# xshazwar/noize-job

Hardware: AMD Instinct MI355X
Metric: Mcells/s 4096^2 simplex13oct->Gauss5x17->FlowMap->Erosion; %HBM roofline @1/8GPU (higher is better)
Workload: dtype f32

## Files before the change

noize_job_amd/csrc/nz_filter.hip:

```cpp
#include <cstdlib>

#include "nz_internal.hpp"

namespace {

constexpr int CT = 256;
constexpr int TW = 128;
__host__ __device__ constexpr int conv_hx(int H) { return (H + 3) & ~3; }
constexpr int TH = 64;

__device__ __forceinline__ int clampi(int v, int lo, int hi) { return v < lo ? lo : (v > hi ? hi : v); }

__device__ __forceinline__ int xcd_tile_index() {
    int bid = blockIdx.x;
    int nb = gridDim.x, q = nb >> 3, r = nb & 7;
    int x = bid & 7, k = bid >> 3;
    return x * q + (x < r ? x : r) + k;
}

__device__ __forceinline__ void tile_origin(const nz_geom &g, int OW, int OH, int &ox0, int &oz0) {
    int tiles_x = (g.cols + OW - 1) / OW;
    int bid = xcd_tile_index();
    int by = bid / tiles_x;
    int bx = bid - by * tiles_x;
    ox0 = bx * OW;
    oz0 = g.or0 + by * OH;
}

constexpr int RB = 8;

__device__ __forceinline__ float dpp_prev(float v) {
    return __builtin_bit_cast(float, __builtin_amdgcn_mov_dpp(__builtin_bit_cast(int, v), 0x138, 0xf, 0xf, true));
}
__device__ __forceinline__ float dpp_next(float v) {
    return __builtin_bit_cast(float, __builtin_amdgcn_mov_dpp(__builtin_bit_cast(int, v), 0x130, 0xf, 0xf, true));
}

#ifdef NZ_CONV_PROBE
__device__ unsigned long long *nz_probe_buf = nullptr;
#define NZ_PB_PARAM , unsigned long long *nz_pb
#define NZ_PB_ARG , nz_pb
#define NZ_PB_INIT unsigned long long *nz_pb = threadIdx.x == 0 ? nz_probe_buf : nullptr
#define NZ_PROBE(slot, val)                                              \
    do {                                                                 \
        if (nz_pb) nz_pb[(size_t)blockIdx.x * 24 + (slot)] = (val);      \
    } while (0)
#define NZ_PROBE_T(slot) NZ_PROBE(slot, __builtin_amdgcn_s_memrealtime())
#else
#define NZ_PB_PARAM
#define NZ_PB_ARG
#define NZ_PB_INIT
#define NZ_PROBE(slot, val)
#define NZ_PROBE_T(slot)
#endif

constexpr int conv_waves(int ks, int nt, int rbt) { return rbt < RB ? 4 : ks == 5 ? 6 : (nt >= 512 || ks >= 7) ? 4 : 6; }
constexpr int conv_nbuf(int o) { return o >= 2 ? 1 : 2; }

typedef unsigned nz_v4u __attribute__((ext_vector_type(4)));
constexpr int NZ_AUX_SC1 = 16;
__device__ __forceinline__ float4 load16_sc1(const float *base, size_t float_off) {
    __amdgpu_buffer_rsrc_t r = __builtin_amdgcn_make_buffer_rsrc(const_cast<float *>(base), 0, -1, 0x00020000);
    nz_v4u t = __builtin_amdgcn_raw_buffer_load_b128(r, (int)(float_off * 4), 0, NZ_AUX_SC1);
    return make_float4(__uint_as_float(t.x), __uint_as_float(t.y), __uint_as_float(t.z), __uint_as_float(t.w));
}
__device__ __forceinline__ void store16_sc1(float *base, size_t float_off, float4 v) {
    __amdgpu_buffer_rsrc_t r = __builtin_amdgcn_make_buffer_rsrc(base, 0, -1, 0x00020000);
    nz_v4u t = {__float_as_uint(v.x), __float_as_uint(v.y), __float_as_uint(v.z), __float_as_uint(v.w)};
    __builtin_amdgcn_raw_buffer_store_b128(t, r, (int)(float_off * 4), 0, NZ_AUX_SC1);
}
__device__ __forceinline__ float load4_sc1(const float *base, size_t float_off) {
    __amdgpu_buffer_rsrc_t r = __builtin_amdgcn_make_buffer_rsrc(const_cast<float *>(base), 0, -1, 0x00020000);
    return __uint_as_float(__builtin_amdgcn_raw_buffer_load_b32(r, (int)(float_off * 4), 0, NZ_AUX_SC1));
}
__device__ __forceinline__ void store4_sc1(float *base, size_t float_off, float v) {
    __amdgpu_buffer_rsrc_t r = __builtin_amdgcn_make_buffer_rsrc(base, 0, -1, 0x00020000);
    __builtin_amdgcn_raw_buffer_store_b32(__float_as_uint(v), r, (int)(float_off * 4), 0, NZ_AUX_SC1);
}

template <bool FAST>
__device__ __forceinline__ float tap_acc(float total, float v, float k) {
    return FAST ? __builtin_fmaf(v, k, total) : total + v * k;
}
template <bool FAST, bool SEED>
__device__ __forceinline__ float tap_first(float v, float k) {
    return FAST ? __builtin_fmaf(v, k, 0.0f) : SEED ? 0.0f + v * k : v * k;
}

template <int KS, bool UNIT, int NT, bool SC1, bool FAST, int RBT>
__device__ __forceinline__ void conv_tile(const float *__restrict__ src, float *__restrict__ dst, const nz_geom &g,
                                          const nz_kernel_taps &taps, int T, int aligned, int ox0, int oz0,
                                          float4 *s_edge_raw NZ_PB_PARAM) {
    constexpr int O = (KS - 1) / 2;
    constexpr int WN = 4 + 2 * O;
    constexpr int ZN = RBT + 2 * O;
    constexpr int TH = NT / 32 * RBT;
    static_assert(O <= RBT, "a block's window reaches into the neighbouring blocks only");
    constexpr int NBUF = conv_nbuf(O);
    float4 (*s_edge)[TH / RBT][2][O][TW / 4] = reinterpret_cast<float4 (*)[TH / RBT][2][O][TW / 4]>(s_edge_raw);

    const int tid = threadIdx.x, cg = tid & 31, rb = tid >> 5;
    const int H = T * O, HX = conv_hx(H);
    const int OW = TW - 2 * HX, OH = TH - 2 * H;
    const int lx0 = ox0 - HX, lz0 = oz0 - H;
    const int gx0 = lx0 + cg * 4, gzb = lz0 + rb * RBT;
    const bool inside = lx0 >= 0 && lx0 + TW <= g.cols && lz0 >= g.zc0 && lz0 + TH - 1 <= g.zc1;
    const bool fast = inside && aligned;
    NZ_PROBE_T(0);
    NZ_PROBE(14, (unsigned long long)__builtin_amdgcn_s_getreg(4 | (0 << 6) | (31 << 11)));
    NZ_PROBE(15, (unsigned long long)__builtin_amdgcn_s_getreg(20 | (0 << 6) | (31 << 11)));

    float v[RBT][4];
    if (fast) {
#pragma unroll
        for (int r = 0; r < RBT; r++) {
            float4 t = SC1 ? load16_sc1(src, (size_t)(gzb + r) * g.pitch + gx0)
                           : *reinterpret_cast<const float4 *>(src + (size_t)(gzb + r) * g.pitch + gx0);
            v[r][0] = t.x; v[r][1] = t.y; v[r][2] = t.z; v[r][3] = t.w;
        }
        asm volatile("; 16-byte loads issued" ::: "memory");
    } else {
        asm volatile("; clamped 4-byte loads of an edge tile" ::: "memory");
#pragma unroll
        for (int r = 0; r < RBT; r++) {
            size_t row = (size_t)clampi(gzb + r, g.zc0, g.zc1) * g.pitch;
#pragma unroll
            for (int e = 0; e < 4; e++) {
                const size_t off = row + clampi(gx0 + e, 0, g.cols - 1);
                v[r][e] = SC1 ? load4_sc1(src, off) : src[off];
            }
        }
    }
#ifdef NZ_CONV_PROBE
    asm volatile("s_waitcnt vmcnt(0)" ::: "memory");
    NZ_PROBE_T(9);
#endif
    const int icx = g.cols - 1 - gx0 + O;
    const int iz0 = g.zc0 - gzb + O, iz1 = g.zc1 - gzb + O;

    for (int t = 0; t < T; t++) {
#pragma unroll
        for (int r = 0; r < RBT; r++) {
            float w[WN];
#pragma unroll
            for (int o = 0; o < O; o++) {
                w[o] = dpp_prev(v[r][4 - O + o]);
                w[4 + O + o] = dpp_next(v[r][o]);
            }
#pragma unroll
            for (int e = 0; e < 4; e++) w[O + e] = v[r][e];
            if (!inside) {
                if (gx0 == 0) {
#pragma unroll
                    for (int o = 0; o < O; o++) w[o] = w[O];
                }
                if (icx >= O && icx < WN - 1) {
                    float wc = w[O];
#pragma unroll
                    for (int i = O + 1; i < WN; i++) wc = (i == icx) ? w[i] : wc;
#pragma unroll
                    for (int i = O + 1; i < WN; i++) w[i] = (i > icx) ? wc : w[i];
                }
            }
#pragma unroll
            for (int e = 0; e < 4; e++) {
                float total = tap_first<FAST, false>(w[e], taps.kx[0]);
#pragma unroll
                for (int kk = 1; kk < KS; kk++) total = tap_acc<FAST>(total, w[e + kk], taps.kx[kk]);
                v[r][e] = UNIT ? total : total * taps.factor;
            }
        }
        const int par = NBUF == 2 ? (t & 1) : 0;
#pragma unroll
        for (int o = 0; o < O; o++) {
            s_edge[par][rb][0][o][cg] = make_float4(v[o][0], v[o][1], v[o][2], v[o][3]);
            s_edge[par][rb][1][o][cg] = make_float4(v[RBT - O + o][0], v[RBT - O + o][1], v[RBT - O + o][2], v[RBT - O + o][3]);
        }
        if (t == 0) NZ_PROBE_T(16);
        __syncthreads();
        if (t == 0) NZ_PROBE_T(17);
        float z[ZN][4];
#pragma unroll
        for (int o = 0; o < O; o++) {
            float4 a = rb > 0 ? s_edge[par][rb - 1][1][o][cg] : make_float4(v[0][0], v[0][1], v[0][2], v[0][3]);
            float4 b = rb < TH / RBT - 1 ? s_edge[par][rb + 1][0][o][cg]
                                        : make_float4(v[RBT - 1][0], v[RBT - 1][1], v[RBT - 1][2], v[RBT - 1][3]);
            z[o][0] = a.x; z[o][1] = a.y; z[o][2] = a.z; z[o][3] = a.w;
            z[RBT + O + o][0] = b.x; z[RBT + O + o][1] = b.y; z[RBT + O + o][2] = b.z; z[RBT + O + o][3] = b.w;
        }
        if (NBUF == 1 && t + 1 < T) __syncthreads();
#pragma unroll
        for (int r = 0; r < RBT; r++)
#pragma unroll
            for (int e = 0; e < 4; e++) z[O + r][e] = v[r][e];
        if (!inside) {
            if (iz0 > 0 && iz0 < ZN) {
#pragma unroll
                for (int e = 0; e < 4; e++) {
                    float c = z[0][e];
#pragma unroll
                    for (int i = 1; i < ZN; i++) c = (i == iz0) ? z[i][e] : c;
#pragma unroll
                    for (int i = 0; i < ZN - 1; i++) z[i][e] = (i < iz0) ? c : z[i][e];
                }
            }
            if (iz1 >= 0 && iz1 < ZN - 1) {
#pragma unroll
                for (int e = 0; e < 4; e++) {
                    float c = z[0][e];
#pragma unroll
                    for (int i = 1; i < ZN; i++) c = (i == iz1) ? z[i][e] : c;
#pragma unroll
                    for (int i = 1; i < ZN; i++) z[i][e] = (i > iz1) ? c : z[i][e];
                }
            }
        }
#pragma unroll
        for (int r = 0; r < RBT; r++) {
#pragma unroll
            for (int e = 0; e < 4; e++) {
                float total = tap_first<FAST, !UNIT>(z[r + 2 * O][e], taps.kz[0]);
#pragma unroll
                for (int kk = 1; kk < KS; kk++) total = tap_acc<FAST>(total, z[r + 2 * O - kk][e], taps.kz[kk]);
                v[r][e] = UNIT ? total : total * taps.factor;
            }
        }
        NZ_PROBE_T(1 + t);
    }

    if constexpr (UNIT && !FAST) {
#pragma unroll
        for (int r = 0; r < RBT; r++)
#pragma unroll
            for (int e = 0; e < 4; e++) v[r][e] += 0.0f;
    }

    if (fast) {
#pragma unroll
        for (int r = 0; r < RBT; r++) {
            int lr = rb * RBT + r, gz = gzb + r;
            bool in = lr >= H && lr < H + OH && cg * 4 >= HX && cg * 4 < HX + OW && gz < g.or1;
            if (in) {
                if (SC1) store16_sc1(dst, (size_t)gz * g.pitch + gx0, make_float4(v[r][0], v[r][1], v[r][2], v[r][3]));
                else *reinterpret_cast<float4 *>(dst + (size_t)gz * g.pitch + gx0) = make_float4(v[r][0], v[r][1], v[r][2], v[r][3]);
            }
        }
    } else {
        asm volatile("; guarded stores of an edge tile" ::: "memory");
#pragma unroll
        for (int r = 0; r < RBT; r++) {
            int lr = rb * RBT + r, gz = gzb + r;
            bool in = lr >= H && lr < H + OH && cg * 4 >= HX && cg * 4 < HX + OW && gz < g.or1 && gx0 < g.cols;
            if (in) {
#pragma unroll
                for (int e = 0; e < 4; e++)
                    if (gx0 + e < g.cols) {
                        if (SC1) store4_sc1(dst, (size_t)gz * g.pitch + gx0 + e, v[r][e]);
                        else dst[(size_t)gz * g.pitch + gx0 + e] = v[r][e];
                    }
            }
        }
    }
    NZ_PROBE_T(12);
}

template <int KS, bool UNIT, int NT, bool FAST, int RBT>
__global__ __launch_bounds__(NT) __attribute__((amdgpu_waves_per_eu(conv_waves(KS, NT, RBT)))) void conv_reg_kernel(const float *__restrict__ src, float *__restrict__ dst, nz_geom g,
                                                     nz_kernel_taps taps, int T, int aligned) {
    constexpr int O = (KS - 1) / 2;
    constexpr int TH = NT / 32 * RBT;
    constexpr int NBUF = conv_nbuf(O);
    __shared__ float4 s_edge[NBUF][TH / RBT][2][O][TW / 4];
    const int H = T * O, HX = conv_hx(H);
    src += blockIdx.y * g.bstride;
    dst += blockIdx.y * g.bstride;
    int ox0, oz0;
    tile_origin(g, TW - 2 * HX, TH - 2 * H, ox0, oz0);
    NZ_PB_INIT;
    conv_tile<KS, UNIT, NT, false, FAST, RBT>(src, dst, g, taps, T, aligned, ox0, oz0, &s_edge[0][0][0][0][0] NZ_PB_ARG);
}

constexpr int NZ_CHAIN_MAXL = 8;
struct nz_chain {
    int L, total;
    int T[NZ_CHAIN_MAXL], first[NZ_CHAIN_MAXL + 1], tiles_x[NZ_CHAIN_MAXL];
    unsigned epoch;
    int *flags;
    float *plane[2];
    int delay_item, delay_sleeps;
    int spin_limit;
    unsigned *err_host;
    unsigned *err_epoch;
};

__host__ __device__ __forceinline__ int chain_class_count(int n, int c) { return n > c ? (n - c + 7) >> 3 : 0; }

template <int KS, bool UNIT, int NT, bool FAST, int RBT>
__global__ __launch_bounds__(NT) __attribute__((amdgpu_waves_per_eu(conv_waves(KS, NT, RBT)))) void conv_chain_kernel(nz_geom g, nz_kernel_taps taps,
                                                                                                                       nz_chain ch, int aligned) {
    constexpr int O = (KS - 1) / 2;
    constexpr int TH = NT / 32 * RBT;
    constexpr int NBUF = conv_nbuf(O);
    __shared__ float4 s_edge[NBUF][TH / RBT][2][O][TW / 4];
    NZ_PB_INIT;
    NZ_PROBE_T(18);
    int l = 0, tile = 0;
    {
        const int vb = blockIdx.x;
        const int cls = vb & 7;
        while (l + 1 < ch.L && vb >= ch.first[l + 1]) l++;
        int start = 0;
        for (int c = 0; c < cls; c++) start += chain_class_count(ch.first[l + 1], c) - chain_class_count(ch.first[l], c);
        const int mine = chain_class_count(ch.first[l + 1], cls) - chain_class_count(ch.first[l], cls);
        const int j = chain_class_count(vb, cls) - chain_class_count(ch.first[l], cls);
        tile = start + ((cls & 1) ? mine - 1 - j : j);
    }
    NZ_PROBE_T(7);
    NZ_PROBE(13, ((unsigned long long)l << 32) | (unsigned)tile);
    const int T = ch.T[l], H = T * O, HX = conv_hx(H);
    const int OW = TW - 2 * HX, OH = TH - 2 * H;
    const int by = tile / ch.tiles_x[l], bx = tile - by * ch.tiles_x[l];
    const int ox0 = bx * OW, oz0 = g.or0 + by * OH;
    if (l > 0) {
        const int Tp = ch.T[l - 1], Hp = Tp * O, HXp = conv_hx(Hp);
        const int OWp = TW - 2 * HXp, OHp = TH - 2 * Hp;
        const int Hw = max(H, Hp), HXw = max(HX, HXp);
        const int ix0 = max(ox0 - HXw, 0), ix1 = min(ox0 + OW + HXw - 1, g.cols - 1);
        const int iz0 = max(oz0 - Hw, g.or0), iz1 = min(oz0 + OH + Hw - 1, g.or1 - 1);
        const int px0 = ix0 / OWp, px1 = ix1 / OWp, py0 = (iz0 - g.or0) / OHp, py1 = (iz1 - g.or0) / OHp;
        const int nx = px1 - px0 + 1, nd = nx * (py1 - py0 + 1);
        if ((int)threadIdx.x < nd) {
            const int dep = (py0 + (int)threadIdx.x / nx) * ch.tiles_x[l - 1] + px0 + (int)threadIdx.x % nx;
            const int *f = ch.flags + ch.first[l - 1] + dep;
            int spins = 0;
            while ((unsigned)__hip_atomic_load(f, __ATOMIC_RELAXED, __HIP_MEMORY_SCOPE_AGENT) != ch.epoch) {
                __builtin_amdgcn_s_sleep(32);
                if (++spins > ch.spin_limit) {
                    atomicMin(ch.err_epoch, ch.epoch);
                    __threadfence();
                    __hip_atomic_store(ch.err_host, 1u, __ATOMIC_RELEASE, __HIP_MEMORY_SCOPE_SYSTEM);
                    break;
                }
            }
        }
        __syncthreads();
    }
    NZ_PROBE_T(8);
    if (ch.first[l] + tile == ch.delay_item)
        for (int i = 0; i < ch.delay_sleeps; i++) __builtin_amdgcn_s_sleep(127);
    conv_tile<KS, UNIT, NT, true, FAST, RBT>(ch.plane[l & 1], ch.plane[(l + 1) & 1], g, taps, T, aligned, ox0, oz0, &s_edge[0][0][0][0][0] NZ_PB_ARG);
    asm volatile("s_waitcnt vmcnt(0)" ::: "memory");
    NZ_PROBE_T(10);
    __syncthreads();
    NZ_PROBE_T(11);
    if (threadIdx.x == 0) {
        __hip_atomic_store(&ch.flags[ch.first[l] + tile], (int)ch.epoch, __ATOMIC_RELAXED, __HIP_MEMORY_SCOPE_AGENT);
    }
}



template <int E>
__global__ __launch_bounds__(CT) void erosion_reg_kernel(const float *__restrict__ src, float *__restrict__ dst,
                                                        nz_geom g, int aligned) {
    __shared__ float4 s_edge[TH / RB][E][TW / 4];
    constexpr float BIG = 3.40282347e+38f;
    constexpr int HX = E > 4 ? 8 : 4;
    static_assert(E >= 1 && E <= RB, "the window reaches one 8-row block / two lanes back at most");
    const int tid = threadIdx.x, cg = tid & 31, rb = tid >> 5;
    const int OW = TW - HX, OH = TH - E;
    src += blockIdx.y * g.bstride;
    dst += blockIdx.y * g.bstride;
    int ox0, oz0;
    tile_origin(g, OW, OH, ox0, oz0);
    const int lx0 = ox0 - HX, lz0 = oz0 - E;
    const int gx0 = lx0 + cg * 4, gzb = lz0 + rb * RB;
    const bool inside = lx0 >= 0 && lx0 + TW <= g.cols && lz0 >= g.zc0 && lz0 + TH - 1 <= g.zc1;
    const bool fast = inside && aligned;
    float v[RB][4];
#pragma unroll
    for (int r = 0; r < RB; r++) {
        int gz = gzb + r;
        if (fast) {
            float4 t = *reinterpret_cast<const float4 *>(src + (size_t)gz * g.pitch + gx0);
            v[r][0] = t.x; v[r][1] = t.y; v[r][2] = t.z; v[r][3] = t.w;
            asm volatile("; 16-byte load" ::: "memory");
        } else {
            bool zin = gz >= g.zc0 && gz <= g.zc1;
#pragma unroll
            for (int e = 0; e < 4; e++) {
                int gx = gx0 + e;
                v[r][e] = (zin && gx >= 0 && gx < g.cols) ? src[(size_t)gz * g.pitch + gx] : BIG;
            }
        }
    }
#pragma unroll
    for (int r = 0; r < RB; r++) {
        float w[4 + E];
        if constexpr (E <= 4) {
#pragma unroll
            for (int o = 0; o < E; o++) w[o] = dpp_prev(v[r][4 - E + o]);
            if (cg == 0) {
#pragma unroll
                for (int o = 0; o < E; o++) w[o] = BIG;
            }
        } else {
            float p1[4];
#pragma unroll
            for (int e = 0; e < 4; e++) {
                float t = dpp_prev(v[r][e]);
                asm volatile("" : "+v"(t));
                p1[e] = cg == 0 ? BIG : t;
            }
#pragma unroll
            for (int o = 0; o < E - 4; o++) {
                float t = dpp_prev(p1[8 - E + o]);
                asm volatile("" : "+v"(t));
                w[o] = cg == 0 ? BIG : t;
            }
#pragma unroll
            for (int e = 0; e < 4; e++) w[E - 4 + e] = p1[e];
        }
#pragma unroll
        for (int e = 0; e < 4; e++) w[E + e] = v[r][e];
#pragma unroll
        for (int e = 0; e < 4; e++) {
            float m = w[e];
#pragma unroll
            for (int k = 1; k <= E; k++) m = fminf(m, w[e + k]);
            v[r][e] = m;
        }
    }
#pragma unroll
    for (int o = 0; o < E; o++)
        s_edge[rb][o][cg] = make_float4(v[RB - E + o][0], v[RB - E + o][1], v[RB - E + o][2], v[RB - E + o][3]);
    __syncthreads();
    float z[RB + E][4];
#pragma unroll
    for (int o = 0; o < E; o++) {
        float4 a = rb > 0 ? s_edge[rb - 1][o][cg] : make_float4(BIG, BIG, BIG, BIG);
        z[o][0] = a.x; z[o][1] = a.y; z[o][2] = a.z; z[o][3] = a.w;
    }
#pragma unroll
    for (int r = 0; r < RB; r++)
#pragma unroll
        for (int e = 0; e < 4; e++) z[E + r][e] = v[r][e];
#pragma unroll
    for (int r = 0; r < RB; r++) {
        int lr = rb * RB + r, gz = gzb + r;
        float out[4];
#pragma unroll
        for (int e = 0; e < 4; e++) {
            float m = z[r][e];
#pragma unroll
            for (int k = 1; k <= E; k++) m = fminf(m, z[r + k][e]);
            out[e] = m;
        }
        bool in = lr >= E && cg * 4 >= HX && gz < g.or1 && gx0 < g.cols;
        if (in) {
            if (aligned && gx0 + 4 <= g.cols) {
                *reinterpret_cast<float4 *>(dst + (size_t)gz * g.pitch + gx0) = make_float4(out[0], out[1], out[2], out[3]);
                asm volatile("; 16-byte store" ::: "memory");
            } else {
#pragma unroll
                for (int e = 0; e < 4; e++)
                    if (gx0 + e < g.cols) dst[(size_t)gz * g.pitch + gx0 + e] = out[e];
            }
        }
    }
}

template <bool FAST>
__global__ __launch_bounds__(CT) void conv_pass_x_kernel(const float *__restrict__ src, float *__restrict__ dst,
                                                        nz_geom g, nz_kernel_taps taps) {
    int x = blockIdx.x * CT + threadIdx.x;
    int z = g.or0 + blockIdx.y;
    if (x >= g.cols || z >= g.or1) return;
    const int k_off = (taps.ksize - 1) / 2;
    const float *row = src + (size_t)z * g.pitch;
    float total = 0.0f;
    for (int k = -k_off; k <= k_off; k++) total = tap_acc<FAST>(total, row[clampi(x + k, 0, g.cols - 1)], taps.kx[k_off + k]);
    dst[(size_t)z * g.pitch + x] = total * taps.factor;
}

template <bool FAST>
__global__ __launch_bounds__(CT) void conv_pass_z_kernel(const float *__restrict__ src, float *__restrict__ dst,
                                                        nz_geom g, nz_kernel_taps taps) {
    int x = blockIdx.x * CT + threadIdx.x;
    int z = g.or0 + blockIdx.y;
    if (x >= g.cols || z >= g.or1) return;
    const int k_off = (taps.ksize - 1) / 2;
    float total = 0.0f;
    for (int k = k_off; k >= -k_off; k--)
        total = tap_acc<FAST>(total, src[(size_t)clampi(z + k, g.zc0, g.zc1) * g.pitch + x], taps.kz[k_off - k]);
    dst[(size_t)z * g.pitch + x] = total * taps.factor;
}

constexpr int WD_W = 128;

template <int O, bool UNIT, int WD_NT, bool FAST>
__global__ __launch_bounds__(WD_NT) void conv_wide_kernel(const float *__restrict__ src, float *__restrict__ dst, nz_geom g,
                                                      nz_kernel_taps taps, int aligned) {
    constexpr int KS = 2 * O + 1;
    constexpr int WD_H = WD_NT / 8;
    constexpr int NR = WD_H + 2 * O;
    constexpr int WD_XH = (WD_NT == 512 && O >= 11) ? 12 : 16;
    constexpr int WD_AP = WD_W + 2 * WD_XH;
    constexpr int OFF = WD_XH - O;
    constexpr int OFA = OFF & ~3, SH = OFF & 3;
    constexpr int NF = (SH + 8 + 2 * O + 3) / 4;
    static_assert(OFA + 8 * 15 + 4 * NF <= WD_AP, "the last thread's X window leaves the staged row");
    __shared__ float4 s_a[NR * WD_AP / 4];
    const int tid = threadIdx.x;
    src += blockIdx.y * g.bstride;
    dst += blockIdx.y * g.bstride;
    const int tiles_x = (g.cols + WD_W - 1) / WD_W;
    const int bid = xcd_tile_index();
    const int by = bid / tiles_x, bx = bid - by * tiles_x;
    const int x0 = bx * WD_W, z0 = g.or0 + by * WD_H;

    const bool inside = aligned && x0 - WD_XH >= 0 && x0 + WD_W + WD_XH <= g.cols && z0 - O >= g.zc0 &&
                        z0 + WD_H + O - 1 <= g.zc1;
    for (int i = tid; i < NR * (WD_AP / 4); i += WD_NT) {
        int r = i / (WD_AP / 4), c4 = i - r * (WD_AP / 4);
        int gx = x0 - WD_XH + 4 * c4;
        float4 t;
        if (inside) {
            t = *reinterpret_cast<const float4 *>(src + (size_t)(z0 - O + r) * g.pitch + gx);
            asm volatile("; 16-byte load" ::: "memory");
        } else {
            const float *row = src + (size_t)clampi(z0 - O + r, g.zc0, g.zc1) * g.pitch;
            t.x = row[clampi(gx, 0, g.cols - 1)];
            t.y = row[clampi(gx + 1, 0, g.cols - 1)];
            t.z = row[clampi(gx + 2, 0, g.cols - 1)];
            t.w = row[clampi(gx + 3, 0, g.cols - 1)];
        }
        s_a[i] = t;
    }
    __syncthreads();

    {
        const int tx = tid & 15, ry = tid >> 4;
        for (int r = ry; r < NR; r += WD_NT / 16) {
            float w[NF * 4];
            const float4 *a = s_a + (r * WD_AP + OFA + 8 * tx) / 4;
#pragma unroll
            for (int f = 0; f < NF; f++) {
                float4 t = a[f];
                w[4 * f] = t.x; w[4 * f + 1] = t.y; w[4 * f + 2] = t.z; w[4 * f + 3] = t.w;
            }
            float o[8];
#pragma unroll
            for (int e = 0; e < 8; e++) {
                float total = tap_first<FAST, false>(w[SH + e], taps.kx[0]);
#pragma unroll
                for (int kk = 1; kk < KS; kk++) total = tap_acc<FAST>(total, w[SH + e + kk], taps.kx[kk]);
                o[e] = UNIT ? total : total * taps.factor;
            }
            float4 *b = s_a + (r * WD_AP + WD_XH + 8 * tx) / 4;
            b[0] = make_float4(o[0], o[1], o[2], o[3]);
            b[1] = make_float4(o[4], o[5], o[6], o[7]);
        }
    }
    __syncthreads();

    if constexpr (WD_NT == 512) {
        const int cg = tid & 63, rg = tid >> 6;
        float v[8 + 2 * O][2];
        const float2 *col = reinterpret_cast<const float2 *>(s_a) + ((rg * 8) * WD_AP + WD_XH) / 2 + cg;
#pragma unroll
        for (int i = 0; i < 8 + 2 * O; i++) {
            float2 t = col[i * (WD_AP / 2)];
            v[i][0] = t.x; v[i][1] = t.y;
        }
        const int gx = x0 + 2 * cg;
#pragma unroll
        for (int j = 0; j < 8; j++) {
            float o[2];
#pragma unroll
            for (int e = 0; e < 2; e++) {
                float total = tap_first<FAST, true>(v[j + 2 * O][e], taps.kz[0]);
#pragma unroll
                for (int kk = 1; kk < KS; kk++) total = tap_acc<FAST>(total, v[j + 2 * O - kk][e], taps.kz[kk]);
                o[e] = UNIT ? total : total * taps.factor;
            }
            int gz = z0 + rg * 8 + j;
            if (gz < g.or1 && gx < g.cols) {
                float *out = dst + (size_t)gz * g.pitch + gx;
                if (aligned && gx + 2 <= g.cols) {
                    *reinterpret_cast<float2 *>(out) = make_float2(o[0], o[1]);
                    asm volatile("; 8-byte store" ::: "memory");
                } else {
                    out[0] = o[0];
                    if (gx + 1 < g.cols) out[1] = o[1];
                }
            }
        }
    } else {
        const int cg = tid & 31, rg = tid >> 5;
        float v[4 + 2 * O][4];
#pragma unroll
        for (int i = 0; i < 4 + 2 * O; i++) {
            float4 t = s_a[((rg * 4 + i) * WD_AP + WD_XH) / 4 + cg];
            v[i][0] = t.x; v[i][1] = t.y; v[i][2] = t.z; v[i][3] = t.w;
        }
        const int gx = x0 + 4 * cg;
#pragma unroll
        for (int j = 0; j < 4; j++) {
            float o[4];
#pragma unroll
            for (int e = 0; e < 4; e++) {
                float total = tap_first<FAST, true>(v[j + 2 * O][e], taps.kz[0]);
#pragma unroll
                for (int kk = 1; kk < KS; kk++) total = tap_acc<FAST>(total, v[j + 2 * O - kk][e], taps.kz[kk]);
                o[e] = UNIT ? total : total * taps.factor;
            }
            int gz = z0 + rg * 4 + j;
            if (gz < g.or1 && gx < g.cols) {
                float *out = dst + (size_t)gz * g.pitch + gx;
                if (aligned && gx + 4 <= g.cols) {
                    *reinterpret_cast<float4 *>(out) = make_float4(o[0], o[1], o[2], o[3]);
                    asm volatile("; 16-byte store" ::: "memory");
                } else {
#pragma unroll
                    for (int e = 0; e < 4; e++)
                        if (gx + e < g.cols) out[e] = o[e];
                }
            }
        }
    }
}

template <int O, int NT>
int32_t launch_wide_nt(hipStream_t s, const float *src, float *dst, const nz_geom &g, const nz_kernel_taps &k) {
    constexpr int WD_H = NT / 8;
    long long blocks = (long long)((g.cols + WD_W - 1) / WD_W) * ((g.or1 - g.or0 + WD_H - 1) / WD_H);
    int aligned = (g.pitch % 4 == 0) && ((reinterpret_cast<uintptr_t>(src) | reinterpret_cast<uintptr_t>(dst)) & 15) == 0;
    nz_with_unit_fast(k, [&](auto unit, auto fast) {
        NZ_LAUNCH((conv_wide_kernel<O, unit, NT, fast>), dim3((unsigned)blocks, g.count), dim3(NT), 0, s, src, dst, g, k, aligned);
    });
    NZ_HIP(hipGetLastError());
    return NZ_OK;
}

template <int O>
int32_t launch_wide(hipStream_t s, const float *src, float *dst, const nz_geom &g, const nz_kernel_taps &k) {
    if constexpr (2 * O + 1 >= 17) return launch_wide_nt<O, 512>(s, src, dst, g, k);
    else return launch_wide_nt<O, 256>(s, src, dst, g, k);
}

constexpr long long CONV_SMALL_CELLS = 7 * 1024 * 1024;
constexpr long long CONV_TINY_CELLS = 600 * 1024;

enum conv_shape { CONV_BIG, CONV_SMALL, CONV_TINY };
constexpr int CONV_SMALL_NT = 512, CONV_SMALL_RB = 4, CONV_TINY_NT = 1024, CONV_TINY_RB = 2;
static_assert(CONV_SMALL_NT / 32 * CONV_SMALL_RB == 64 && CONV_TINY_NT / 32 * CONV_TINY_RB == 64,
              "the hosts size a small grid's tiles as 64 rows (nz_conv_max_fused, the fusion caps of nz_stages.cpp)");

static bool conv_small_grid(int ksize, const nz_geom &g) {
    if (ksize < 5) return false;
    static const int env = getenv("NZ_CONV_SMALL") ? atoi(getenv("NZ_CONV_SMALL")) : 1;
    if (env == 0) return false;
    if (env == 2) return true;
    return (long long)g.cols * (g.or1 - g.or0) * g.count < CONV_SMALL_CELLS;
}
static conv_shape conv_shape_of(int ksize, const nz_geom &g) {
    if (!conv_small_grid(ksize, g)) return CONV_BIG;
    return ksize == 5 && (long long)g.cols * (g.or1 - g.or0) * g.count <= CONV_TINY_CELLS ? CONV_TINY : CONV_SMALL;
}

template <int KS, class F>
auto with_conv_shape(conv_shape sh, F &&f) {
    using std::integral_constant;
    if constexpr (KS == 5)
        if (sh == CONV_TINY) return f(integral_constant<int, CONV_TINY_NT>(), integral_constant<int, CONV_TINY_RB>());
    if (sh != CONV_BIG) return f(integral_constant<int, CONV_SMALL_NT>(), integral_constant<int, CONV_SMALL_RB>());
    return f(integral_constant<int, (KS >= 5 ? 512 : 256)>(), integral_constant<int, RB>());
}

struct conv_tiling { int x, y; };
template <int KS, int NT, int RBT>
conv_tiling conv_tiles(const nz_geom &g, int T) {
    constexpr int O = (KS - 1) / 2, RTH = NT / 32 * RBT;
    const int H = T * O, HX = conv_hx(H);
    const int OW = TW - 2 * HX, OH = RTH - 2 * H;
    return {(g.cols + OW - 1) / OW, (g.or1 - g.or0 + OH - 1) / OH};
}

template <int KS, int NT, int RBT>
int32_t launch_fused_nt(hipStream_t s, const float *src, float *dst, const nz_geom &g, const nz_kernel_taps &k, int T) {
    const conv_tiling t = conv_tiles<KS, NT, RBT>(g, T);
    const long long blocks = (long long)t.x * t.y;
    int aligned = ((reinterpret_cast<uintptr_t>(src) | reinterpret_cast<uintptr_t>(dst) | (uintptr_t)(g.pitch * 4)) & 15) == 0;
    nz_with_unit_fast(k, [&](auto unit, auto fast) {
        NZ_LAUNCH((conv_reg_kernel<KS, unit, NT, fast, RBT>), dim3((unsigned)blocks, g.count), dim3(NT), 0, s, src, dst, g, k, T, aligned);
    });
    NZ_HIP(hipGetLastError());
    return NZ_OK;
}

template <int KS>
int32_t launch_fused(hipStream_t s, const float *src, float *dst, const nz_geom &g, const nz_kernel_taps &k, int T) {
    return with_conv_shape<KS>(conv_shape_of(KS, g), [&](auto nt, auto rbt) { return launch_fused_nt<KS, nt, rbt>(s, src, dst, g, k, T); });
}

int g_chain_delay_item = -1, g_chain_delay_sleeps = 0;
int g_chain_spin_limit = 1 << 21;

template <int KS, int NT, int RBT>
nz_chain conv_chain_plan(const nz_geom &g, const int *Ts, int L) {
    nz_chain ch{};
    ch.L = L;
    for (int l = 0; l < L; l++) {
        const conv_tiling t = conv_tiles<KS, NT, RBT>(g, Ts[l]);
        ch.T[l] = Ts[l];
        ch.tiles_x[l] = t.x;
        ch.first[l + 1] = ch.first[l] + t.x * t.y;
    }
    ch.total = ch.first[L];
    return ch;
}

template <int KS, int NT, int RBT>
int32_t launch_chain_nt(hipStream_t s, float *plane0, float *plane1, const nz_geom &g, const nz_kernel_taps &k, const int *Ts,
                        int L, int *flags, unsigned epoch, unsigned *err_host, unsigned *err_epoch) {
    nz_chain ch = conv_chain_plan<KS, NT, RBT>(g, Ts, L);
    ch.epoch = epoch;
    ch.flags = flags;
    ch.plane[0] = plane0;
    ch.plane[1] = plane1;
    ch.delay_item = g_chain_delay_item;
    ch.delay_sleeps = g_chain_delay_sleeps;
    ch.spin_limit = g_chain_spin_limit;
    ch.err_host = err_host;
    ch.err_epoch = err_epoch;
    int aligned = ((reinterpret_cast<uintptr_t>(plane0) | reinterpret_cast<uintptr_t>(plane1) | (uintptr_t)(g.pitch * 4)) & 15) == 0;
    nz_with_unit_fast(k, [&](auto unit, auto fast) {
        NZ_LAUNCH((conv_chain_kernel<KS, unit, NT, fast, RBT>), dim3((unsigned)ch.total), dim3(NT), 0, s, g, k, ch, aligned);
    });
    NZ_HIP(hipGetLastError());
    return NZ_OK;
}

template <int KS>
int32_t launch_chain(hipStream_t s, float *plane0, float *plane1, const nz_geom &g, const nz_kernel_taps &k, const int *Ts,
                     int L, int *flags, unsigned epoch, unsigned *err_host, unsigned *err_epoch) {
    return with_conv_shape<KS>(conv_shape_of(KS, g), [&](auto nt, auto rbt) {
        return launch_chain_nt<KS, nt, rbt>(s, plane0, plane1, g, k, Ts, L, flags, epoch, err_host, err_epoch);
    });
}

template <int KS>
int chain_items(const nz_geom &g, const int *Ts, int L) {
    return with_conv_shape<KS>(conv_shape_of(KS, g), [&](auto nt, auto rbt) { return conv_chain_plan<KS, nt, rbt>(g, Ts, L).total; });
}

}

bool nz_conv_small_grid(int ksize, const nz_geom &g) { return conv_small_grid(ksize, g); }
bool nz_conv_tiny_grid(int ksize, const nz_geom &g) { return conv_shape_of(ksize, g) == CONV_TINY; }

int nz_conv_chain_items(int ksize, const nz_geom &g, const int *Ts, int L) {
    if (L < 1 || L > NZ_CHAIN_MAXL) return 0;
    switch (ksize) {
        case 3: return chain_items<3>(g, Ts, L);
        case 5: return chain_items<5>(g, Ts, L);
        case 7: return chain_items<7>(g, Ts, L);
        case 9: return chain_items<9>(g, Ts, L);
    }
    return 0;
}

int32_t nz_launch_conv_chain(hipStream_t s, float *plane0, float *plane1, const nz_geom &g, const nz_kernel_taps &k,
                             const int *Ts, int L, int *flags, unsigned epoch, unsigned *err_host, unsigned *err_epoch) {
    if (L < 1 || L > NZ_CHAIN_MAXL || g.count != 1 || (size_t)g.rows * g.pitch * 4 >= ((size_t)1 << 32)) {
        nz_set_error("conv_chain: %d launches / %d grids / plane of %zu bytes unsupported", L, g.count, (size_t)g.rows * g.pitch * 4);
        return NZ_ERR_INVALID;
    }
    for (int l = 0; l < L; l++)
        if (Ts[l] < 1 || Ts[l] > nz_conv_max_fused(k.ksize)) {
            nz_set_error("conv_chain: T=%d unsupported for kernelSize %d", Ts[l], k.ksize);
            return NZ_ERR_INVALID;
        }
    if (g.or1 <= g.or0) return NZ_OK;
    switch (k.ksize) {
        case 3: return launch_chain<3>(s, plane0, plane1, g, k, Ts, L, flags, epoch, err_host, err_epoch);
        case 5: return launch_chain<5>(s, plane0, plane1, g, k, Ts, L, flags, epoch, err_host, err_epoch);
        case 7: return launch_chain<7>(s, plane0, plane1, g, k, Ts, L, flags, epoch, err_host, err_epoch);
        case 9: return launch_chain<9>(s, plane0, plane1, g, k, Ts, L, flags, epoch, err_host, err_epoch);
    }
    return NZ_ERR_INVALID;
}

int nz_conv_max_fused(int ksize) {
    switch (ksize) {
        case 3: return 8;
        case 5: return 9;
        case 7: return 5;
        case 9: return 4;
        default: return 0;
    }
}

int32_t nz_launch_conv_fused(hipStream_t s, const float *src, float *dst, const nz_geom &g,
                             const nz_kernel_taps &k, int T) {
    if (T < 1 || T > nz_conv_max_fused(k.ksize)) {
        nz_set_error("conv_fused: T=%d unsupported for kernelSize %d", T, k.ksize);
        return NZ_ERR_INVALID;
    }
    if (g.or1 <= g.or0) return NZ_OK;
    if (nz_conv_stream_wanted(g, k.ksize, T)) return nz_launch_conv_stream(s, src, dst, g, k, T);
    switch (k.ksize) {
        case 3: return launch_fused<3>(s, src, dst, g, k, T);
        case 5: return launch_fused<5>(s, src, dst, g, k, T);
        case 7: return launch_fused<7>(s, src, dst, g, k, T);
        case 9: return launch_fused<9>(s, src, dst, g, k, T);
    }
    return NZ_ERR_INVALID;
}

bool nz_conv_has_wide(int ksize) { return (ksize & 1) && ksize >= 11 && ksize <= 25; }

int32_t nz_launch_conv_wide(hipStream_t s, const float *src, float *dst, const nz_geom &g, const nz_kernel_taps &k) {
    if (g.or1 <= g.or0) return NZ_OK;
    switch (k.ksize) {
        case 11: return launch_wide<5>(s, src, dst, g, k);
        case 13: return launch_wide<6>(s, src, dst, g, k);
        case 15: return launch_wide<7>(s, src, dst, g, k);
        case 17: return launch_wide<8>(s, src, dst, g, k);
        case 19: return launch_wide<9>(s, src, dst, g, k);
        case 21: return launch_wide<10>(s, src, dst, g, k);
        case 23: return launch_wide<11>(s, src, dst, g, k);
        case 25: return launch_wide<12>(s, src, dst, g, k);
    }
    nz_set_error("conv_wide: kernelSize %d unsupported", k.ksize);
    return NZ_ERR_INVALID;
}

int32_t nz_launch_conv_pass_x(hipStream_t s, const float *src, float *dst, const nz_geom &g,
                              const nz_kernel_taps &k) {
    if (g.or1 <= g.or0) return NZ_OK;
    dim3 grid((g.cols + CT - 1) / CT, g.or1 - g.or0);
    if (nz_tls_float_mode >= NZ_FLOAT_FAST) hipLaunchKernelGGL(conv_pass_x_kernel<true>, grid, dim3(CT), 0, s, src, dst, g, k);
    else hipLaunchKernelGGL(conv_pass_x_kernel<false>, grid, dim3(CT), 0, s, src, dst, g, k);
    NZ_HIP(hipGetLastError());
    return NZ_OK;
}

int32_t nz_launch_conv_pass_z(hipStream_t s, const float *src, float *dst, const nz_geom &g,
                              const nz_kernel_taps &k) {
    if (g.or1 <= g.or0) return NZ_OK;
    dim3 grid((g.cols + CT - 1) / CT, g.or1 - g.or0);
    if (nz_tls_float_mode >= NZ_FLOAT_FAST) hipLaunchKernelGGL(conv_pass_z_kernel<true>, grid, dim3(CT), 0, s, src, dst, g, k);
    else hipLaunchKernelGGL(conv_pass_z_kernel<false>, grid, dim3(CT), 0, s, src, dst, g, k);
    NZ_HIP(hipGetLastError());
    return NZ_OK;
}

int nz_erosion_max_fused() {
    static const int cap = getenv("NZ_EROSION_EMAX") ? atoi(getenv("NZ_EROSION_EMAX")) : 8;
    return cap < 1 ? 1 : (cap > 8 ? 8 : cap);
}

int32_t nz_launch_erosion_fused(hipStream_t s, const float *src, float *dst, const nz_geom &g, int E) {
    if (E < 1 || E > nz_erosion_max_fused()) {
        nz_set_error("erosion_fused: E=%d unsupported", E);
        return NZ_ERR_INVALID;
    }
    if (g.or1 <= g.or0) return NZ_OK;
    int OW = TW - (E > 4 ? 8 : 4), OH = TH - E;
    long long blocks = (long long)((g.cols + OW - 1) / OW) * ((g.or1 - g.or0 + OH - 1) / OH);
    int aligned = ((reinterpret_cast<uintptr_t>(src) | reinterpret_cast<uintptr_t>(dst) | (uintptr_t)(g.pitch * 4)) & 15) == 0;
    switch (E) {
        case 1: NZ_LAUNCH((erosion_reg_kernel<1>), dim3((unsigned)blocks, g.count), dim3(CT), 0, s, src, dst, g, aligned); break;
        case 2: NZ_LAUNCH((erosion_reg_kernel<2>), dim3((unsigned)blocks, g.count), dim3(CT), 0, s, src, dst, g, aligned); break;
        case 3: NZ_LAUNCH((erosion_reg_kernel<3>), dim3((unsigned)blocks, g.count), dim3(CT), 0, s, src, dst, g, aligned); break;
        case 4: NZ_LAUNCH((erosion_reg_kernel<4>), dim3((unsigned)blocks, g.count), dim3(CT), 0, s, src, dst, g, aligned); break;
        case 5: NZ_LAUNCH((erosion_reg_kernel<5>), dim3((unsigned)blocks, g.count), dim3(CT), 0, s, src, dst, g, aligned); break;
        case 6: NZ_LAUNCH((erosion_reg_kernel<6>), dim3((unsigned)blocks, g.count), dim3(CT), 0, s, src, dst, g, aligned); break;
        case 7: NZ_LAUNCH((erosion_reg_kernel<7>), dim3((unsigned)blocks, g.count), dim3(CT), 0, s, src, dst, g, aligned); break;
        default: NZ_LAUNCH((erosion_reg_kernel<8>), dim3((unsigned)blocks, g.count), dim3(CT), 0, s, src, dst, g, aligned); break;
    }
    NZ_HIP(hipGetLastError());
    return NZ_OK;
}

#ifdef NZ_CONV_PROBE
extern "C" int32_t nz_debug_set_conv_probe(void *buf) {
    return hipMemcpyToSymbol(HIP_SYMBOL(nz_probe_buf), &buf, sizeof buf) == hipSuccess ? 0 : -3;
}
#endif

extern "C" int32_t nz_debug_chain_delay(int32_t item, int32_t sleeps) {
    g_chain_delay_item = item;
    g_chain_delay_sleeps = sleeps < 0 ? 0 : sleeps;
    return NZ_OK;
}

extern "C" int32_t nz_debug_chain_poll_limit(int32_t polls) {
    g_chain_spin_limit = polls > 0 ? polls : 1 << 21;
    return NZ_OK;
}
```

Before: 27170.

## Split 5-tap 512-thread conv into interior and register-lean edge paths

```diff
diff --git a/noize_job_amd/csrc/nz_filter.hip b/noize_job_amd/csrc/nz_filter.hip
--- a/noize_job_amd/csrc/nz_filter.hip
+++ b/noize_job_amd/csrc/nz_filter.hip
@@ -54,8 +54,17 @@
 #define NZ_PROBE_T(slot)
 #endif
 
-constexpr int conv_waves(int ks, int nt, int rbt) { return rbt < RB ? 4 : ks == 5 ? 6 : (nt >= 512 || ks >= 7) ? 4 : 6; }
+constexpr bool conv_split(int ks, int nt, int rbt) { return ks == 5 && nt == 512 && rbt == RB; }
+constexpr int conv_edge_rows(int ks, int nt, int rbt) { return nt / 32 * rbt / 2 + (ks - 1) / 2; }
+constexpr int conv_waves(int ks, int nt, int rbt) { return rbt < RB ? 4 : conv_split(ks, nt, rbt) ? 8 : ks == 5 ? 6 : (nt >= 512 || ks >= 7) ? 4 : 6; }
 constexpr int conv_nbuf(int o) { return o >= 2 ? 1 : 2; }
+constexpr int conv_lds_f4(int ks, int nt, int rbt) {
+    const int o = (ks - 1) / 2, xch = conv_nbuf(o) * (nt / 32) * 2 * o * (TW / 4);
+    if (!conv_split(ks, nt, rbt)) return xch;
+    const int xch_split = xch + 2 * o * (TW / 4), staged = conv_edge_rows(ks, nt, rbt) * (TW / 4);
+    return xch_split > staged ? xch_split : staged;
+}
+static_assert(4 * conv_lds_f4(5, 512, RB) * 16 <= 160 * 1024, "four big 5-tap workgroups share a CU's 160 KB of LDS");
 
 typedef unsigned nz_v4u __attribute__((ext_vector_type(4)));
 constexpr int NZ_AUX_SC1 = 16;
@@ -85,6 +94,281 @@
 template <bool FAST, bool SEED>
 __device__ __forceinline__ float tap_first(float v, float k) {
     return FAST ? __builtin_fmaf(v, k, 0.0f) : SEED ? 0.0f + v * k : v * k;
+}
+
+__device__ __forceinline__ int conv_lane_here() {
+    unsigned m = ~0u;
+    asm volatile("" : "+s"(m));
+    return (int)__builtin_amdgcn_mbcnt_hi(m, __builtin_amdgcn_mbcnt_lo(m, 0u));
+}
+
+template <int KS, bool UNIT, int NT, bool SC1, bool FAST, int RBT>
+__device__ __forceinline__ void conv_tile_interior(const float *__restrict__ src, float *__restrict__ dst, const nz_geom &g,
+                                                   const nz_kernel_taps &taps, int T, int aligned, int ox0, int oz0, int wave,
+                                                   float4 *s_edge_raw NZ_PB_PARAM) {
+    constexpr int O = (KS - 1) / 2;
+    constexpr int WN = 4 + 2 * O;
+    constexpr int ZN = RBT + 2 * O;
+    constexpr int TH = NT / 32 * RBT, NB = TH / RBT;
+    static_assert(conv_nbuf(O) == 1, "one edge buffer");
+    const int tid = threadIdx.x, cg = tid & 31, rb = tid >> 5;
+    const int H = T * O, HX = conv_hx(H);
+    const int OW = TW - 2 * HX, OH = TH - 2 * H;
+    const int gx0 = ox0 - HX + cg * 4, gzb = oz0 - H + rb * RBT;
+
+    float v[RBT][4];
+    if (aligned) {
+#pragma unroll
+        for (int r = 0; r < RBT; r++) {
+            float4 t = SC1 ? load16_sc1(src, (size_t)(gzb + r) * g.pitch + gx0)
+                           : *reinterpret_cast<const float4 *>(src + (size_t)(gzb + r) * g.pitch + gx0);
+            v[r][0] = t.x; v[r][1] = t.y; v[r][2] = t.z; v[r][3] = t.w;
+        }
+        asm volatile("; 16-byte loads issued" ::: "memory");
+    } else {
+        asm volatile("; 4-byte loads of an unaligned plane" ::: "memory");
+#pragma unroll
+        for (int r = 0; r < RBT; r++) {
+            const size_t off = (size_t)(gzb + r) * g.pitch + gx0;
+#pragma unroll
+            for (int e = 0; e < 4; e++) v[r][e] = SC1 ? load4_sc1(src, off + e) : src[off + e];
+        }
+    }
+#ifdef NZ_CONV_PROBE
+    asm volatile("s_waitcnt vmcnt(0)" ::: "memory");
+    NZ_PROBE_T(9);
+#endif
+    if (rb == 0 || rb == NB - 1) {
+        float4 (*s_end)[O][TW / 4] = reinterpret_cast<float4 (*)[O][TW / 4]>(s_edge_raw) + (rb == 0 ? 0 : 2 * NB + 1);
+#pragma unroll
+        for (int o = 0; o < O; o++) s_end[0][o][cg] = make_float4(0.0f, 0.0f, 0.0f, 0.0f);
+    }
+
+    for (int t = 0; t < T; t++) {
+#pragma unroll
+        for (int r = 0; r < RBT; r++) {
+            float w[WN];
+#pragma unroll
+            for (int o = 0; o < O; o++) {
+                w[o] = dpp_prev(v[r][4 - O + o]);
+                w[4 + O + o] = dpp_next(v[r][o]);
+            }
+#pragma unroll
+            for (int e = 0; e < 4; e++) w[O + e] = v[r][e];
+#pragma unroll
+            for (int e = 0; e < 4; e++) {
+                float total = tap_first<FAST, false>(w[e], taps.kx[0]);
+#pragma unroll
+                for (int kk = 1; kk < KS; kk++) total = tap_acc<FAST>(total, w[e + kk], taps.kx[kk]);
+                v[r][e] = UNIT ? total : total * taps.factor;
+            }
+            __builtin_amdgcn_sched_barrier(0);
+        }
+        __syncthreads();
+        const int lane = conv_lane_here();
+        float4 (*s_edge)[O][TW / 4] = reinterpret_cast<float4 (*)[O][TW / 4]>(s_edge_raw) + 2 * (2 * wave + (lane >> 5));
+        const int cg = lane & 31;
+#pragma unroll
+        for (int o = 0; o < O; o++) {
+            s_edge[1][o][cg] = make_float4(v[o][0], v[o][1], v[o][2], v[o][3]);
+            s_edge[2][o][cg] = make_float4(v[RBT - O + o][0], v[RBT - O + o][1], v[RBT - O + o][2], v[RBT - O + o][3]);
+        }
+        if (t == 0) NZ_PROBE_T(16);
+        __syncthreads();
+        if (t == 0) NZ_PROBE_T(17);
+        float z[ZN][4];
+#pragma unroll
+        for (int o = 0; o < O; o++) {
+            float4 a = s_edge[0][o][cg];
+            float4 b = s_edge[3][o][cg];
+            z[o][0] = a.x; z[o][1] = a.y; z[o][2] = a.z; z[o][3] = a.w;
+            z[RBT + O + o][0] = b.x; z[RBT + O + o][1] = b.y; z[RBT + O + o][2] = b.z; z[RBT + O + o][3] = b.w;
+        }
+#pragma unroll
+        for (int r = 0; r < RBT; r++)
+#pragma unroll
+            for (int e = 0; e < 4; e++) z[O + r][e] = v[r][e];
+#pragma unroll
+        for (int r = 0; r < RBT; r++) {
+#pragma unroll
+            for (int e = 0; e < 4; e++) {
+                float total = tap_first<FAST, !UNIT>(z[r + 2 * O][e], taps.kz[0]);
+#pragma unroll
+                for (int kk = 1; kk < KS; kk++) total = tap_acc<FAST>(total, z[r + 2 * O - kk][e], taps.kz[kk]);
+                v[r][e] = UNIT ? total : total * taps.factor;
+            }
+            __builtin_amdgcn_sched_barrier(0);
+        }
+        NZ_PROBE_T(1 + t);
+    }
+
+    if constexpr (UNIT && !FAST) {
+#pragma unroll
+        for (int r = 0; r < RBT; r++)
+#pragma unroll
+            for (int e = 0; e < 4; e++) v[r][e] += 0.0f;
+    }
+
+    const int tid_st = wave * 64 + conv_lane_here();
+    const int cg_st = tid_st & 31, rb_st = tid_st >> 5;
+    const int gx_st = ox0 - HX + cg_st * 4, gz_st = oz0 - H + rb_st * RBT;
+#pragma unroll
+    for (int r = 0; r < RBT; r++) {
+        int lr = rb_st * RBT + r, gz = gz_st + r;
+        bool in = lr >= H && lr < H + OH && cg_st * 4 >= HX && cg_st * 4 < HX + OW && gz < g.or1;
+        if (in) {
+            if (aligned) {
+                if (SC1) store16_sc1(dst, (size_t)gz * g.pitch + gx_st, make_float4(v[r][0], v[r][1], v[r][2], v[r][3]));
+                else *reinterpret_cast<float4 *>(dst + (size_t)gz * g.pitch + gx_st) = make_float4(v[r][0], v[r][1], v[r][2], v[r][3]);
+            } else {
+#pragma unroll
+                for (int e = 0; e < 4; e++) {
+                    if (SC1) store4_sc1(dst, (size_t)gz * g.pitch + gx_st + e, v[r][e]);
+                    else dst[(size_t)gz * g.pitch + gx_st + e] = v[r][e];
+                }
+            }
+        }
+    }
+    NZ_PROBE_T(12);
+}
+
+template <int RBT>
+__device__ __forceinline__ void conv_rotate_rows(float (&v)[RBT][4], const float (&last)[4]) {
+    float l[4] = {last[0], last[1], last[2], last[3]};
+#pragma unroll
+    for (int r = 0; r + 1 < RBT; r++)
+#pragma unroll
+        for (int e = 0; e < 4; e++) v[r][e] = v[r + 1][e];
+#pragma unroll
+    for (int e = 0; e < 4; e++) v[RBT - 1][e] = l[e];
+}
+
+template <int KS, bool UNIT, int NT, bool SC1, bool FAST, int RBT>
+__device__ __forceinline__ void conv_tile_edge(const float *__restrict__ src, float *__restrict__ dst, const nz_geom &g,
+                                               const nz_kernel_taps &taps, int T, int ox0, int oz0, int wave,
+                                               float4 *s_raw NZ_PB_PARAM) {
+    constexpr int O = (KS - 1) / 2;
+    constexpr int WN = 4 + 2 * O;
+    constexpr int TH = NT / 32 * RBT, NB = TH / RBT;
+    constexpr int ER = conv_edge_rows(KS, NT, RBT);
+    float *s_f = reinterpret_cast<float *>(s_raw);
+
+    const int H = T * O, HX = conv_hx(H);
+    const int OW = TW - 2 * HX, OH = TH - 2 * H;
+    const int lx0 = ox0 - HX, lz0 = oz0 - H;
+    const int c_lo = max(-lx0, 0), c_hi = min(g.cols - 1 - lx0, TW - 1);
+    const int r_lo = max(g.zc0 - lz0, 0), r_hi = min(g.zc1 - lz0, TH - 1);
+#define NZ_EDGE_THREAD const int tid = wave * 64 + conv_lane_here(), cg = tid & 31, rb = tid >> 5
+
+    float v[RBT][4] = {};
+    asm volatile("; clamped 4-byte loads of an edge tile" ::: "memory");
+#pragma unroll 1
+    for (int r = 0; r < RBT; r++) {
+        NZ_EDGE_THREAD;
+        const size_t row = (size_t)clampi(lz0 + rb * RBT + r, g.zc0, g.zc1) * g.pitch;
+        float t[4];
+#pragma unroll
+        for (int e = 0; e < 4; e++) {
+            const size_t off = row + clampi(lx0 + cg * 4 + e, 0, g.cols - 1);
+            t[e] = SC1 ? load4_sc1(src, off) : src[off];
+        }
+        conv_rotate_rows<RBT>(v, t);
+    }
+#ifdef NZ_CONV_PROBE
+    asm volatile("s_waitcnt vmcnt(0)" ::: "memory");
+    NZ_PROBE_T(9);
+#endif
+
+    for (int t = 0; t < T; t++) {
+        if (t > 0) __syncthreads();
+#pragma unroll 1
+        for (int r = 0; r < RBT; r++) {
+            NZ_EDGE_THREAD;
+            s_raw[rb * (TW / 4) + cg] = make_float4(v[0][0], v[0][1], v[0][2], v[0][3]);
+            __builtin_amdgcn_fence(__ATOMIC_RELEASE, "wavefront");
+            __builtin_amdgcn_wave_barrier();
+            __builtin_amdgcn_fence(__ATOMIC_ACQUIRE, "wavefront");
+            float w[WN];
+#pragma unroll
+            for (int i = 0; i < WN; i++) w[i] = s_f[rb * TW + clampi(cg * 4 - O + i, c_lo, c_hi)];
+            __builtin_amdgcn_fence(__ATOMIC_RELEASE, "wavefront");
+            __builtin_amdgcn_wave_barrier();
+            float out[4];
+#pragma unroll
+            for (int e = 0; e < 4; e++) {
+                float total = tap_first<FAST, false>(w[e], taps.kx[0]);
+#pragma unroll
+                for (int kk = 1; kk < KS; kk++) total = tap_acc<FAST>(total, w[e + kk], taps.kx[kk]);
+                out[e] = UNIT ? total : total * taps.factor;
+            }
+            conv_rotate_rows<RBT>(v, out);
+        }
+        if (t == 0) NZ_PROBE_T(16);
+        __syncthreads();
+        if (t == 0) NZ_PROBE_T(17);
+#pragma unroll 1
+        for (int p = 0; p < 2; p++) {
+            if (p) __syncthreads();
+            {
+                NZ_EDGE_THREAD;
+#pragma unroll
+                for (int r = 0; r < RBT; r++) {
+                    const int lr = rb * RBT + r;
+                    if ((lr >= ER) == (p == 1)) s_raw[(lr - p * ER) * (TW / 4) + cg] = make_float4(v[r][0], v[r][1], v[r][2], v[r][3]);
+                }
+            }
+            __syncthreads();
+            if ((wave >= NB / 4) == (p == 1)) {
+                const int w_lo = p ? TH / 2 - O : 0, w_hi = p ? TH - 1 : ER - 1;
+#pragma unroll 1
+                for (int r = 0; r < RBT; r++) {
+                    NZ_EDGE_THREAD;
+                    const int lr = rb * RBT + r;
+                    float out[4];
+#pragma unroll
+                    for (int kk = 0; kk < KS; kk++) {
+                        int row = clampi(clampi(lr + O - kk, r_lo, r_hi), w_lo, w_hi);
+                        row = row >= ER && p ? row - ER : row;
+                        const float4 zr = s_raw[row * (TW / 4) + cg];
+                        const float zv[4] = {zr.x, zr.y, zr.z, zr.w};
+#pragma unroll
+                        for (int e = 0; e < 4; e++)
+                            out[e] = kk == 0 ? tap_first<FAST, !UNIT>(zv[e], taps.kz[0]) : tap_acc<FAST>(out[e], zv[e], taps.kz[kk]);
+                    }
+#pragma unroll
+                    for (int e = 0; e < 4; e++) out[e] = UNIT ? out[e] : out[e] * taps.factor;
+                    conv_rotate_rows<RBT>(v, out);
+                }
+            }
+        }
+        NZ_PROBE_T(1 + t);
+    }
+
+    if constexpr (UNIT && !FAST) {
+#pragma unroll
+        for (int r = 0; r < RBT; r++)
+#pragma unroll
+            for (int e = 0; e < 4; e++) v[r][e] += 0.0f;
+    }
+
+    asm volatile("; guarded stores of an edge tile" ::: "memory");
+#pragma unroll 1
+    for (int r = 0; r < RBT; r++) {
+        NZ_EDGE_THREAD;
+        const int lr = rb * RBT + r, gz = lz0 + lr, gx0 = lx0 + cg * 4;
+        const bool in = lr >= H && lr < H + OH && cg * 4 >= HX && cg * 4 < HX + OW && gz < g.or1 && gx0 < g.cols;
+        if (in) {
+#pragma unroll
+            for (int e = 0; e < 4; e++)
+                if (gx0 + e < g.cols) {
+                    if (SC1) store4_sc1(dst, (size_t)gz * g.pitch + gx0 + e, v[0][e]);
+                    else dst[(size_t)gz * g.pitch + gx0 + e] = v[0][e];
+                }
+        }
+        conv_rotate_rows<RBT>(v, v[0]);
+    }
+#undef NZ_EDGE_THREAD
+    NZ_PROBE_T(12);
 }
 
 template <int KS, bool UNIT, int NT, bool SC1, bool FAST, int RBT>
@@ -109,6 +393,13 @@
     NZ_PROBE_T(0);
     NZ_PROBE(14, (unsigned long long)__builtin_amdgcn_s_getreg(4 | (0 << 6) | (31 << 11)));
     NZ_PROBE(15, (unsigned long long)__builtin_amdgcn_s_getreg(20 | (0 << 6) | (31 << 11)));
+    if constexpr (conv_split(KS, NT, RBT)) {
+        int wave = __builtin_amdgcn_readfirstlane(tid >> 6);
+        asm volatile("" : "+s"(wave));
+        if (inside) conv_tile_interior<KS, UNIT, NT, SC1, FAST, RBT>(src, dst, g, taps, T, aligned, ox0, oz0, wave, s_edge_raw NZ_PB_ARG);
+        else conv_tile_edge<KS, UNIT, NT, SC1, FAST, RBT>(src, dst, g, taps, T, ox0, oz0, wave, s_edge_raw NZ_PB_ARG);
+        return;
+    }
 
     float v[RBT][4];
     if (fast) {
@@ -269,15 +560,14 @@
                                                      nz_kernel_taps taps, int T, int aligned) {
     constexpr int O = (KS - 1) / 2;
     constexpr int TH = NT / 32 * RBT;
-    constexpr int NBUF = conv_nbuf(O);
-    __shared__ float4 s_edge[NBUF][TH / RBT][2][O][TW / 4];
+    __shared__ float4 s_edge[conv_lds_f4(KS, NT, RBT)];
     const int H = T * O, HX = conv_hx(H);
     src += blockIdx.y * g.bstride;
     dst += blockIdx.y * g.bstride;
     int ox0, oz0;
     tile_origin(g, TW - 2 * HX, TH - 2 * H, ox0, oz0);
     NZ_PB_INIT;
-    conv_tile<KS, UNIT, NT, false, FAST, RBT>(src, dst, g, taps, T, aligned, ox0, oz0, &s_edge[0][0][0][0][0] NZ_PB_ARG);
+    conv_tile<KS, UNIT, NT, false, FAST, RBT>(src, dst, g, taps, T, aligned, ox0, oz0, s_edge NZ_PB_ARG);
 }
 
 constexpr int NZ_CHAIN_MAXL = 8;
@@ -300,10 +590,11 @@
                                                                                                                        nz_chain ch, int aligned) {
     constexpr int O = (KS - 1) / 2;
     constexpr int TH = NT / 32 * RBT;
-    constexpr int NBUF = conv_nbuf(O);
-    __shared__ float4 s_edge[NBUF][TH / RBT][2][O][TW / 4];
+    __shared__ float4 s_edge[conv_lds_f4(KS, NT, RBT)];
     NZ_PB_INIT;
     NZ_PROBE_T(18);
+    int wave0 = __builtin_amdgcn_readfirstlane(threadIdx.x);
+    asm volatile("" : "+s"(wave0));
     int l = 0, tile = 0;
     {
         const int vb = blockIdx.x;
@@ -348,12 +639,14 @@
     NZ_PROBE_T(8);
     if (ch.first[l] + tile == ch.delay_item)
         for (int i = 0; i < ch.delay_sleeps; i++) __builtin_amdgcn_s_sleep(127);
-    conv_tile<KS, UNIT, NT, true, FAST, RBT>(ch.plane[l & 1], ch.plane[(l + 1) & 1], g, taps, T, aligned, ox0, oz0, &s_edge[0][0][0][0][0] NZ_PB_ARG);
+    conv_tile<KS, UNIT, NT, true, FAST, RBT>(ch.plane[l & 1], ch.plane[(l + 1) & 1], g, taps, T, aligned, ox0, oz0, s_edge NZ_PB_ARG);
     asm volatile("s_waitcnt vmcnt(0)" ::: "memory");
     NZ_PROBE_T(10);
     __syncthreads();
     NZ_PROBE_T(11);
-    if (threadIdx.x == 0) {
+    bool first = threadIdx.x == 0;
+    if constexpr (conv_split(KS, NT, RBT)) first = wave0 == 0 && conv_lane_here() == 0;
+    if (first) {
         __hip_atomic_store(&ch.flags[ch.first[l] + tile], (int)ch.epoch, __ATOMIC_RELAXED, __HIP_MEMORY_SCOPE_AGENT);
     }
 }
```

Result: slower. 22920 (-15.6%).
